# facebookresearch/spdl

Measured on AMD Instinct MI355X. Metric: images/sec device-resident JPEG→RGB224, 1/2/4/8×MI355X; % HBM roofline, higher is better.
Workload: dtype u8; 1 GPU; configs[1]: synthetic 480x640 q90 4:2:0 baseline JPEG resident in HBM -> RGB 224x224 u8 (scale bicubic decrease + centred pad, rgb24); global_batch=256, per_gpu_batch=256, distinct_images=32, lanes=4, hw_queues=4, entropy_threads=256, entropy_piece_bytes=131072

## Files before the change

### spdl_amd/csrc/hj_common.h

```cpp
#pragma once
#include <stddef.h>
#include <stdint.h>

#ifndef HJ_HD
#define HJ_HD __host__ __device__
#endif

namespace hj {

constexpr int kMaxComp = 4;

enum { kColorGray = 0, kColorYcbcr, kColorRgb, kColorCmyk, kColorYcck, kColorYcbcrk };
inline HJ_HD bool frame_color(int ncomp, const int32_t* h, const int32_t* v, const int* ids,
                              int adobe, int32_t* color) {
  bool all11 = true;
  for (int c = 0; c < ncomp; c++) all11 = all11 && h[c] == 1 && v[c] == 1;
  if (ncomp == 1) {
    *color = kColorGray;
  } else if (ncomp == 3) {
    const bool rgb = adobe == 0 || (ids[0] == 'R' && ids[1] == 'G' && ids[2] == 'B');
    if (rgb && !all11) return false;
    *color = rgb ? kColorRgb : kColorYcbcr;
  } else {
    if (!all11) return false;
    *color = adobe == 0 ? kColorCmyk : adobe == 2 ? kColorYcck : kColorYcbcrk;
  }
  return true;
}
constexpr int kMaxBpm = 10;
constexpr int kLutBits = 10;
constexpr int kLutSize = 1 << kLutBits;
constexpr int kDcBias = 1024;

constexpr int kMaxSlots = 2048;
constexpr int kRecPad = 4;
constexpr int kMaxEntropyThreads = 1024;

constexpr int kMaxPieces = 64;
constexpr int kChainGranules = 16;
constexpr int kChainHead = 32;
enum ChainSlot {
  kChG0 = 0, kChG1, kChL0, kChL1, kChT,
  kChE0, kChE1, kChB,
  kChDc = 8,
};
enum ChainTag : uint32_t { kTagRec1 = 1, kTagRec2 = 2, kTagDc = 3, kTagFail = 0xFA11u };
inline HJ_HD uint32_t slot_bits(uint32_t maxbits, int sub_bits, uint32_t budget = kMaxSlots) {
  uint32_t need = (uint32_t)(((uint64_t)maxbits + budget - 1) / budget);
  need = (need + 31) & ~31u;
  const uint32_t n = (uint32_t)sub_bits;
  return need > n ? need : n;
}

constexpr uint32_t kKindSlow = 0;
constexpr uint32_t kKindCode = 1;
constexpr uint32_t kKindFull = 2;
constexpr uint32_t kKindSub = 3;
constexpr int kSubBits = 16 - kLutBits;
#ifndef HJ_SUB_POOL
#define HJ_SUB_POOL 2048
#endif
constexpr int kSubPool = HJ_SUB_POOL;

#ifndef HJ_FUSED_THREADS
#define HJ_FUSED_THREADS 256
#endif
constexpr int kFusedThreads = HJ_FUSED_THREADS;
constexpr int kMaxSub = 16;
constexpr int kEntHiShift = 21;

inline HJ_HD uint32_t hj_entry(uint32_t kind, int len, int sym, bool is_dc, int v) {
  const int size = is_dc ? sym : (sym & 15);
  const int run = is_dc ? 0 : (sym >> 4);
  uint32_t zinc, coef = 0, bad = 0;
  if (is_dc || size) {
    zinc = (uint32_t)run + 1u;
    coef = 1;
  } else if (run == 15) {
    zinc = 16;
  } else {
    zinc = 64;
    bad = run != 0;
  }
  const uint32_t sz = kind == kKindFull ? 0u : (uint32_t)size;
  return ((uint32_t)len + sz) | (kind << 5) | (sz << 7) | (zinc << 12) | (coef << 19) | (bad << 20) |
         (((uint32_t)v & 0x7FFu) << kEntHiShift);
}

struct HuffTable {
  uint32_t lut[kLutSize];
  uint32_t sub[kMaxSub << kSubBits];
  int32_t nsub;
  int32_t long_slow;
  int32_t sub_lo;
  int32_t maxcode[18];
  int32_t valoff[17];
  uint8_t vals[256];
};

enum { kSwsX = 0, kSwsOne = 1, kSwsTwo = 2 };
enum SwsTable { kHlPos = 0, kHlCoef, kHcPos, kHcCoef, kVlPos, kVlCoef, kVcPos, kVcCoef, kVmode, kSwsTables };
struct SwsDesc {
  int32_t sw, sh;
  int32_t chr_w;
  int32_t full, gray;
  int32_t hl_taps, hc_taps, vl_taps, vc_taps;
  int32_t hl_size, hc_size, vl_size, vc_size;
  int32_t off[kSwsTables];
  int32_t rb;
  int32_t col_chunk;
  int32_t gbr;
  int32_t pre, pre_rl, pre_rc;
  int32_t yuv, hsub, vsub, chr_h;
};

struct ImageDesc {
  int64_t in_off;
  int64_t in_size;
  int64_t coef_off;
  int64_t plane_off[kMaxComp];
  int64_t seg_off;
  int64_t out_off;
  int64_t wt_off;
  int32_t seg_cap;
  int32_t width, height, ncomp;
  int32_t h_samp[kMaxComp], v_samp[kMaxComp];
  int32_t nblocks;
  int32_t plane_stride[kMaxComp];
  int32_t dx, dy, ow, oh;
  SwsDesc sws;
  int64_t ds_off;
  int32_t ds_cap;
  int32_t color;
  int64_t rec_off;
  int64_t rec_cap;
  int32_t pieces;
  int32_t chain_off;
  int32_t ds_wg0, idct_wg0;
  int32_t hs_wg0, hs_wgs;
  int32_t sws_wg0, sws_bands, sws_chunks;
  int64_t hbuf_off;
  int32_t refuse;
  int32_t idct_blocks;
  int32_t reg_mx0, reg_my0, reg_mw, reg_mh;
  uint32_t reg_mw_magic;
  int32_t win_x[kMaxComp], win_y[kMaxComp], win_w[kMaxComp], win_h[kMaxComp];
  int32_t src;
};

#ifndef HJ_SWS_LDS_KB
#define HJ_SWS_LDS_KB 32
#endif
constexpr int kSwsLdsBudget = HJ_SWS_LDS_KB * 1024;
constexpr int kSwsMaxCols = 256;
inline HJ_HD int sws_col_stride(int rows) { return 2 * (((rows + 5) >> 1) | 1); }

struct ImageInfo {
  int32_t status;
  int32_t width, height, ncomp, hmax, vmax, mcux, mcuy, bpm, nblocks, ri;
  int32_t scan_start;
  int32_t comp_h[kMaxComp], comp_v[kMaxComp];
  int32_t comp_bw[kMaxComp], comp_bh[kMaxComp];
  int32_t comp_w[kMaxComp], comp_hpx[kMaxComp];
  int32_t mcu_comp[kMaxBpm], mcu_dx[kMaxBpm], mcu_dy[kMaxBpm];
  int32_t dc_tab[kMaxComp], ac_tab[kMaxComp];
  uint16_t qt[kMaxComp][64];
  int32_t nseg;
  int32_t clean_len;
// ... 128 lines not shown
```

### spdl_amd/csrc/hj_kernels.hip

```cpp
#include <hip/hip_fp16.h>
#include <hip/hip_runtime.h>

#include "hj_common.h"
#include "hj_destuff.h"
#include "hj_idct.h"
#include "hj_launch.h"
#include "hj_sws_tile.h"

namespace hj {

__device__ __forceinline__ uint32_t rfl(uint32_t v) { return __builtin_amdgcn_readfirstlane(v); }


struct ParseScratch {
  ImageInfo info;
  uint16_t qt[4][64];
  uint8_t bits[8][17];
  uint8_t vals[8][256];
  int32_t have[8];
  int32_t qhave[4];
  int32_t maxcode[8][18];
  int32_t valoff[8][17];
  int32_t dqt_off[4], dqt_pq[4];
  int32_t dht_off[8], dht_n[8];
// ... 302 lines not shown
          k += s.bits[t][l];
          s.maxcode[t][l] = code - 1;
        } else {
          s.maxcode[t][l] = -1;
          s.valoff[t][l] = 0;
        }
        code <<= 1;
      }
      s.maxcode[t][17] = 0x7FFFFFFF;
    }
  }
  __syncthreads();
  HJ_PT();
  if (st != kOk) {
    if (tid == 0) infos[img] = s.info;
    return;
  }
  {
    const Bytes file{bytes + dd.in_off, (lds_u8*)hdr, nh};
    for (int i = tid; i < 8 * 256; i += blockDim.x) {
      const int t = i >> 8, k = i & 255;
      if (s.have[t]) s.vals[t][k] = k < s.dht_n[t] ? file[s.dht_off[t] + k] : 0;
    }
    for (int i = tid; i < 4 * 64; i += blockDim.x) {
      const int t = i >> 6, k = i & 63;
      if (s.qhave[t])
        s.qt[t][k] = s.dqt_pq[t] ? (uint16_t)((file[s.dqt_off[t] + 2 * k] << 8) |
                                              file[s.dqt_off[t] + 2 * k + 1])
                                 : file[s.dqt_off[t] + k];
    }
  }
  __syncthreads();
  HJ_PT();
  for (int i = tid; i < s.info.ncomp * 64; i += blockDim.x)
    s.info.qt[i / 64][i % 64] = s.qt[s.qtsel[i / 64]][i % 64];
  __syncthreads();
  if (s.info.multiscan) {
    if (tid == 0) infos[img] = s.info;
    return;
  }
  __shared__ int tab_nsub[8], tab_slow;
  if (tid == 0) tab_slow = 0;
  __syncthreads();
  if (tid < 8) {
    const int t = tid;
    int nsub = 0;
    if (s.have[t]) {
      uint32_t h = 2166136261u;
      for (int l = 1; l <= 16; l++) h = (h ^ s.bits[t][l]) * 16777619u;
      for (int k = 0; k < s.dht_n[t]; k++) h = (h ^ s.vals[t][k]) * 16777619u;
      s.info.tab_off[t] = s.dht_off[t] - 16;
      s.info.tab_n[t] = s.dht_n[t];
      s.info.tab_hash[t] = h;
      int p_lo = kLutSize, p_hi = -1;
      for (int l = kLutBits + 1; l <= 16; l++) {
        if (s.bits[t][l] == 0) continue;
        const int first = s.maxcode[t][l] - s.bits[t][l] + 1;
        p_lo = min(p_lo, first >> (l - kLutBits));
        p_hi = max(p_hi, s.maxcode[t][l] >> (l - kLutBits));
      }
      nsub = p_hi >= p_lo ? p_hi - p_lo + 1 : 0;
      if (nsub > kMaxSub) {
        atomicOr(&tab_slow, 1 << t);
        nsub = 0;
      }
    } else {
      s.info.tab_off[t] = 0;
      s.info.tab_n[t] = 0;
      s.info.tab_hash[t] = 0;
    }
    s.info.lut_ref[t] = img * 8 + t;
    tab_nsub[t] = nsub;
  }
  __syncthreads();
  if (tid == 0) {
    int ns = 0, seen = 0, subs = 0, slow = 0;
    for (int c = 0; c < s.info.ncomp; c++)
      for (int k = 0; k < 2; k++) {
        const int slot = k == 0 ? s.info.dc_tab[c] : 4 + s.info.ac_tab[c];
        if (!(seen & (1 << slot))) {
          ns++;
          subs += tab_nsub[slot];
          slow |= (tab_slow >> slot) & 1;
        }
        seen |= 1 << slot;
      }
    s.info.ent_wide = !(ns <= 4 && (subs << kSubBits) <= kSubPool && !slow);
  }
  __syncthreads();
  HJ_PT();
#if HJ_PARSE_PROF
  if (tid == 0)
    for (int i = 1; i < npt && i < 8; i++) s.info.sdiag[39 + i] = (int32_t)(pt[i] - pt[0]);
#endif
  static_assert(sizeof(ImageInfo) % 4 == 0, "ImageInfo copied in words");
  {
    const uint32_t* src = reinterpret_cast<const uint32_t*>(&s.info);
    uint32_t* dst = reinterpret_cast<uint32_t*>(infos + img);
    for (int i = tid; i < (int)(sizeof(ImageInfo) / 4); i += blockDim.x) dst[i] = src[i];
  }
}


__global__ void __launch_bounds__(256) lut_kernel(const uint8_t* __restrict__ bytes,
                                                  const ImageDesc* __restrict__ desc,
                                                  ImageInfo* __restrict__ infos,
                                                  HuffTable* __restrict__ luts) {
  __shared__ int first, same, maxcode[18], valoff[17];
  __shared__ uint8_t bits[17], vals[256];
  const int t = blockIdx.x, img = blockIdx.y, tid = threadIdx.x;
  const ImageInfo& in = infos[img];
  if (in.status != kOk || in.multiscan || in.tab_n[t] == 0) return;
  const uint32_t h = in.tab_hash[t];
  const int n = in.tab_n[t];
  const uint8_t* d = bytes + desc[img].in_off + in.tab_off[t];
  if (tid == 0) first = img;
  __syncthreads();
  for (int j = tid; j < img; j += blockDim.x) {
    const ImageInfo& o = infos[j];
    if (o.status == kOk && !o.multiscan && o.tab_n[t] == n && o.tab_hash[t] == h)
      atomicMin(&first, j);
  }
  __syncthreads();
  const int j = first;
  if (j < img) {
    if (tid == 0) same = 1;
    __syncthreads();
    const uint8_t* e = bytes + desc[j].in_off + infos[j].tab_off[t];
    for (int k = tid; k < 16 + n; k += blockDim.x)
      if (d[k] != e[k]) same = 0;
    __syncthreads();
    if (same) {
      if (tid == 0) infos[img].lut_ref[t] = j * 8 + t;
      return;
    }
  }
  if (tid < 16) bits[tid + 1] = d[tid];
  for (int k = tid; k < 256; k += blockDim.x) vals[k] = k < n ? d[16 + k] : 0;
  __syncthreads();
  if (tid == 0) {
    int code = 0, k = 0;
    for (int l = 1; l <= 16; l++) {
      if (bits[l]) {
        valoff[l] = k - code;
        code += bits[l];
        k += bits[l];
        maxcode[l] = code - 1;
      } else {
        maxcode[l] = -1;
        valoff[l] = 0;
      }
      code <<= 1;
    }
    maxcode[17] = 0x7FFFFFFF;
  }
  __syncthreads();
  HuffTable& T = luts[(size_t)img * 8 + t];
  const bool is_dc = t < 4;
  int p_lo = kLutSize, p_hi = -1;
  for (int l = kLutBits + 1; l <= 16; l++) {
    if (bits[l] == 0) continue;
    const int fc = maxcode[l] - bits[l] + 1;
    p_lo = min(p_lo, fc >> (l - kLutBits));
    p_hi = max(p_hi, maxcode[l] >> (l - kLutBits));
  }
  const int nsub = p_hi >= p_lo ? p_hi - p_lo + 1 : 0;
// ... 265 lines not shown
#pragma unroll
    for (int i = 0; i < 5; i++) atomicOr(q + i, x[i]);
  }
  __syncthreads();
  stage_to_global(out, stage, tk, tid);
  if (k == last) {
    const int clen = c.keep_pre + tk;
    if (tid < 64) out[tk + tid] = 0;
    if (tid == 0) {
      infos[img].clean_len = clen;
      infos[img].nseg = min(c.rst_pre + tr + 1, dd.seg_cap);
      sg[0] = 0;
    }
  }
}


typedef unsigned short hj_u16x2 __attribute__((ext_vector_type(2)));
__device__ __forceinline__ uint32_t pk_mul_lo16(uint32_t a, uint32_t b) {
  return __builtin_bit_cast(uint32_t,
                            __builtin_bit_cast(hj_u16x2, a) * __builtin_bit_cast(hj_u16x2, b));
}

constexpr int kMaxTabs = 2 * kMaxComp;
__constant__ uint8_t kSlotOrder[64] = {
    0,  4,  8,  16, 12, 1,  5,  9,  20, 24, 32, 28, 17, 13, 2,  6,  10, 21, 25, 36, 40, 48,
    44, 33, 29, 18, 14, 3,  7,  11, 22, 26, 37, 41, 52, 56, 60, 49, 45, 34, 30, 19, 15, 23,
    27, 38, 42, 53, 57, 61, 50, 46, 35, 31, 39, 43, 54, 58, 62, 51, 47, 55, 59, 63};
#ifndef HJ_WIN_WORDS
#define HJ_WIN_WORDS 12
#endif
constexpr int kWinWords = HJ_WIN_WORDS;

template <int NT, int NTAB>
struct EntShared {
  static constexpr int kTabs = NTAB;
  uint32_t lut[NTAB][kLutSize];
  uint32_t sub[kSubPool];
  int32_t maxcode[NTAB][18];
  int32_t valoff[NTAB][17];
  uint8_t vals[NTAB][256];
  uint32_t run_pos[NT];
  uint32_t run_zb[NT];
  uint32_t qdc[kMaxComp];
  union {
    uint32_t win[kWinWords][NT];
    struct {
      int32_t scan_flag[NT];
      int32_t scan_v[NT][kMaxComp];
      int32_t red[NT];
    } sc;
  };
  int32_t flag;
  int32_t err;
  uint64_t cmask[NT / 64], hmask[NT / 64];
  uint32_t chain_bits;
#if HJ_OWN_CHECK
  uint32_t own_viol;
#endif
  uint32_t chain_sweeps;
  uint32_t left_pos, left_zb;
  int32_t lb_ok, lb_blocks;
  int32_t lb_dc[kMaxComp];
  const HuffTable* gtab;
  int32_t gslot[kMaxTabs];
};
static_assert(sizeof(EntShared<512, 4>) <= 160 * 1024 / 2,
              "entropy LDS must allow 2 workgroups per CU");
static_assert(sizeof(EntShared<256, 4>) <= 160 * 1024 / 3,
              "entropy LDS must allow 3 workgroups per CU at 256 threads");

struct Dec {
  uint32_t wbit;
  uint32_t pos;
  uint32_t z;
  uint32_t bs;
};

struct TabMap {
  uint32_t dmap;
  uint32_t amap;
  uint32_t cmap;
  uint32_t bs_end;
  uint64_t soff;
};

template <int NT>
__device__ __forceinline__ void win_stage(uint32_t* win, const uint32_t* words, uint32_t wb) {
  static_assert(kWinWords % 4 == 0, "window is staged in uint4 units");
  typedef uint32_t u32x4 __attribute__((ext_vector_type(4), aligned(4)));
  const u32x4* src = reinterpret_cast<const u32x4*>(words + wb);
  u32x4 q[kWinWords / 4];
#pragma unroll
  for (int i = 0; i < kWinWords / 4; i++) q[i] = src[i];
#pragma unroll
  for (int i = 0; i < kWinWords / 4; i++) {
    win[(kWinWords - 1 - 4 * i) * NT] = __builtin_bswap32(q[i].x);
    win[(kWinWords - 2 - 4 * i) * NT] = __builtin_bswap32(q[i].y);
    win[(kWinWords - 3 - 4 * i) * NT] = __builtin_bswap32(q[i].z);
    win[(kWinWords - 4 - 4 * i) * NT] = __builtin_bswap32(q[i].w);
  }
}

template <int NT>
__device__ __forceinline__ void dec_init(Dec& d, uint32_t* win, const uint32_t* words, uint32_t p,
                                         uint32_t z, uint32_t bs) {
  d.wbit = p & ~31u;
  win_stage<NT>(win, words, p >> 5);
  d.pos = p;
  d.z = z;
  d.bs = bs;
}

template <int NT>
__device__ __forceinline__ uint32_t dec_peek(Dec& d, uint32_t* win, const uint32_t* words) {
  uint32_t rel = d.pos - d.wbit;
  if (__any(rel >= 32u * (kWinWords - 1))) {
    d.wbit = d.pos & ~31u;
    win_stage<NT>(win, words, d.pos >> 5);
    rel = d.pos - d.wbit;
  }
  const uint32_t* pw = win + (kWinWords - 2 - (int)(rel >> 5)) * NT;
  const uint64_t lohi = (uint64_t)pw[0] | ((uint64_t)pw[NT] << 32);
  return (uint32_t)((lohi << (rel & 31u)) >> 32);
}

__device__ __forceinline__ void dec_skip(Dec& d, uint32_t nbits) { d.pos += nbits; }

template <int NT>
__device__ __forceinline__ uint32_t dec_peek3(Dec& d, uint32_t* win, const uint32_t* words,
                                              uint64_t& p01, uint64_t& p12) {
  uint32_t rel = d.pos - d.wbit;
  if (__any(rel >= 32u * (kWinWords - 2))) {
    d.wbit = d.pos & ~31u;
    win_stage<NT>(win, words, d.pos >> 5);
    rel = d.pos - d.wbit;
  }
  const uint32_t* pw = win + (kWinWords - 3 - (int)(rel >> 5)) * NT;
  const uint32_t w2 = pw[0], w1 = pw[NT], w0 = pw[2 * NT];
  p01 = (uint64_t)w1 | ((uint64_t)w0 << 32);
  p12 = (uint64_t)w2 | ((uint64_t)w1 << 32);
  return rel & 31u;
}

__device__ __forceinline__ uint32_t tab_slot(const TabMap& m, const Dec& d, bool is_dc) {
  return __builtin_amdgcn_ubfe(is_dc ? m.dmap : m.amap, d.bs, 3);
}
__device__ __forceinline__ uint32_t next_bs(const TabMap& m, uint32_t bs) {
  return bs + 3u == m.bs_end ? 0u : bs + 3u;
}

template <class SH>
__device__ __attribute__((noinline)) uint32_t slow_symbol(const SH& S, int t, uint32_t hi,
                                                          bool is_dc) {
  const bool g = t >= SH::kTabs;
  const HuffTable* G = g ? S.gtab + S.gslot[t] : nullptr;
  const int tl = g ? 0 : t;
  const uint32_t w16 = hi >> 16;
  for (int l = 1; l <= 16; l++) {
    const int code = (int)(w16 >> (16 - l));
    if (code <= (g ? G->maxcode[l] : S.maxcode[tl][l])) {
      const int sym = g ? G->vals[G->valoff[l] + code] : S.vals[tl][S.valoff[tl][l] + code];
      if (is_dc && sym > 15) return 1;
      return hj_entry(kKindCode, l, sym, is_dc, 0);
    }
  }
  return 1;
}

template <bool SLOW, class SH>
__device__ __forceinline__ uint32_t lookup(const SH& S, uint32_t t, uint32_t hi, bool is_dc,
                                           uint64_t soff) {
  if constexpr (SLOW) {
    if (t >= (uint32_t)SH::kTabs) {
      const HuffTable& G = S.gtab[S.gslot[t]];
      uint32_t e = G.lut[hi >> (32 - kLutBits)];
      if (((e >> 5) & 3) == kKindSub)
        e = G.sub[((e >> kEntHiShift) << kSubBits) |
                  ((hi >> (32 - kLutBits - kSubBits)) & ((1u << kSubBits) - 1))];
      if (((e >> 5) & 3) == kKindSlow) e = slow_symbol(S, (int)t, hi, is_dc);
      return e;
    }
  }
  uint32_t e = S.lut[t][hi >> (32 - kLutBits)];
  if constexpr (!SLOW) {
    const uint32_t a2 = ((hi >> 16) + (uint32_t)(soff >> (16u * t))) & (uint32_t)(kSubPool - 1);
    const uint32_t e2 = S.sub[a2];
    return ((e >> 5) & 3) == kKindSub ? e2 : e;
  }
  if (((e >> 5) & 3) == kKindSub)
    e = S.sub[((e >> kEntHiShift) << kSubBits) |
              ((hi >> (32 - kLutBits - kSubBits)) & ((1u << kSubBits) - 1))];
  if constexpr (SLOW) {
    if (((e >> 5) & 3) == kKindSlow) e = slow_symbol(S, (int)t, hi, is_dc);
  }
  return e;
}

template <bool SLOW, class SH>
__device__ __forceinline__ uint32_t lookup_fast(const SH& S, uint32_t t, uint32_t hi,
                                                uint64_t soff) {
  if constexpr (SLOW) {
    if (t >= (uint32_t)SH::kTabs) {
      const HuffTable& G = S.gtab[S.gslot[t]];
      uint32_t e = G.lut[hi >> (32 - kLutBits)];
      if (((e >> 5) & 3) == kKindSub)
        e = G.sub[((e >> kEntHiShift) << kSubBits) |
                  ((hi >> (32 - kLutBits - kSubBits)) & ((1u << kSubBits) - 1))];
      return e;
    }
    uint32_t e = S.lut[t][hi >> (32 - kLutBits)];
    if (((e >> 5) & 3) == kKindSub)
      e = S.sub[((e >> kEntHiShift) << kSubBits) |
                ((hi >> (32 - kLutBits - kSubBits)) & ((1u << kSubBits) - 1))];
    return e;
  } else {
    return lookup<false>(S, t, hi, false, soff);
  }
}

template <int NT, bool SLOW, class SH>
__device__ int decode_state(const SH& S, Dec& d, uint32_t* win, const uint32_t* words,
                            const TabMap& m, const uint32_t end) {
  int nend = 0;
  const int open0 = d.z != 0u;
  while (d.pos < end) {
    uint64_t p01, p12;
    const uint32_t r = dec_peek3<NT>(d, win, words, p01, p12);
    uint32_t nbits;
    {
      const uint32_t hi = (uint32_t)((p01 << r) >> 32);
      const uint32_t z = d.z;
      const uint32_t t = tab_slot(m, d, z == 0u);
      const uint32_t e = lookup<SLOW>(S, t, hi, z == 0u, m.soff);
      nbits = e & 31u;
      dec_skip(d, nbits);
      const uint32_t zn = z + __builtin_amdgcn_ubfe(e, 12, 7);
      const bool bend = zn >= 64u;
      nend += bend ? 1 : 0;
      const uint32_t bsn = next_bs(m, d.bs);
      d.z = bend ? 0u : zn;
      d.bs = bend ? bsn : d.bs;
    }
    {
      const bool more = d.pos < end;
      const uint32_t r2 = r + nbits;
      const uint64_t pr = r2 < 32u ? p01 : p12;
      const uint32_t hi = (uint32_t)((pr << (r2 & 31u)) >> 32);
      const uint32_t z = d.z;
      const uint32_t t = tab_slot(m, d, z == 0u);
      const uint32_t e = lookup<SLOW>(S, t, hi, z == 0u, m.soff);
      const uint32_t n2 = more ? (e & 31u) : 0u;
      dec_skip(d, n2);
      const uint32_t zn = z + __builtin_amdgcn_ubfe(e, 12, 7);
      const bool bend = more && zn >= 64u;
      nend += bend ? 1 : 0;
      const uint32_t bsn = next_bs(m, d.bs);
      d.z = bend ? 0u : (more ? zn : z);
      d.bs = bend ? bsn : d.bs;
    }
  }
  return nend + (d.z != 0u ? 1 : 0) - open0;
}

template <int NT, bool SLOW, class SH>
__device__ void skip_open_block(const SH& S, Dec& d, uint32_t* win, const uint32_t* words,
                                const TabMap& m, const uint32_t seg_end) {
  while (d.z != 0u && d.pos < seg_end) {
    const uint32_t hi = dec_peek<NT>(d, win, words);
    const uint32_t z = d.z;
    const uint32_t e = lookup<SLOW>(S, tab_slot(m, d, false), hi, false, m.soff);
    const uint32_t nbits = e & 31u;
    dec_skip(d, nbits);
    const uint32_t zn = z + __builtin_amdgcn_ubfe(e, 12, 7);
    const bool bend = zn >= 64u;
    const uint32_t bsn = next_bs(m, d.bs);
    d.z = bend ? 0u : zn;
    d.bs = bend ? bsn : d.bs;
  }
}


__device__ __forceinline__ int sym_value(uint32_t e, uint32_t hi, uint32_t nbits, uint32_t sz) {
  const uint32_t raw = __builtin_amdgcn_ubfe(hi, 32u - nbits, sz);
  const uint32_t top = (uint32_t)__builtin_amdgcn_sbfe((int)raw, sz - 1u, 1);
  const uint32_t neg = ~top & ((1u << sz) - 1u);
  return ((int32_t)e >> kEntHiShift) + (int)(raw - neg);
}

#ifndef HJ_DESC_PAIRS
#define HJ_DESC_PAIRS 0
#endif
struct BlockOut {
  uint32_t* ents;
  uint2* bdesc;
  uint32_t cur;
  uint32_t last;
  uint32_t nblk;
  uint32_t bstart;
  int dcv;
  bool open;
  uint32_t pk[4];
#if HJ_DESC_PAIRS
  uint2 held;
  int hblk;
#endif
#if HJ_OWN_CHECK
  int lo, hi;
  uint32_t viol;
#endif
#if HJ_ABLATIONS
  bool no_list, no_desc;
#endif
};

__device__ __forceinline__ void put_entry(BlockOut& o, uint32_t e, bool put) {
  o.pk[0] = put ? o.pk[1] : o.pk[0];
  o.pk[1] = put ? o.pk[2] : o.pk[1];
  o.pk[2] = put ? o.pk[3] : o.pk[2];
  o.pk[3] = put ? e : o.pk[3];
#if HJ_ABLATIONS
  if (o.no_list) return;
#endif
  if (put && (o.cur & 3u) == 3u) {
    const uint32_t base = min(o.cur & ~3u, o.last & ~3u);
    *reinterpret_cast<uint4*>(o.ents + base) = make_uint4(o.pk[0], o.pk[1], o.pk[2], o.pk[3]);
  }
}

__device__ __forceinline__ void close_block(BlockOut& o, int blk) {
#if HJ_ABLATIONS
  if (o.no_desc) blk = -1;
#endif
  if ((uint32_t)blk < o.nblk) {
#if HJ_OWN_CHECK
    o.viol += (blk < o.lo || blk >= o.hi) ? 1u : 0u;
#endif
    const uint2 dv = make_uint2(o.bstart, (o.cur - o.bstart) | ((uint32_t)o.dcv << 16));
#if HJ_DESC_PAIRS
    uint2* p = o.bdesc + blk;
    const bool hi = ((uintptr_t)p & 8u) != 0;
    if (hi && o.hblk >= 0 && o.hblk == blk - 1) {
      *reinterpret_cast<uint4*>(p - 1) = make_uint4(o.held.x, o.held.y, dv.x, dv.y);
      o.hblk = -1;
    } else {
      if (o.hblk >= 0) o.bdesc[o.hblk] = o.held;
      if (hi) {
        *p = dv;
        o.hblk = -1;
      } else {
        o.held = dv;
        o.hblk = blk;
      }
    }
#else
    o.bdesc[blk] = dv;
#endif
  }
  o.open = false;
}

__device__ __forceinline__ void flush_desc(BlockOut& o) {
#if HJ_DESC_PAIRS
  if (o.hblk >= 0) o.bdesc[o.hblk] = o.held;
  o.hblk = -1;
#endif
}

__device__ __forceinline__ void flush_tail(BlockOut& o) {
  const uint32_t r = o.cur & 3u;
  if (r == 0u) return;
#if HJ_ABLATIONS
  if (o.no_list) return;
#endif
  const uint32_t base = min(o.cur & ~3u, o.last & ~3u);
  const uint32_t m1 = 0u - (uint32_t)(r == 1u), m2 = 0u - (uint32_t)(r == 2u);
  const uint32_t m3 = ~(m1 | m2);
  uint4 q;
  q.x = (o.pk[3] & m1) | (o.pk[2] & m2) | (o.pk[1] & m3);
  q.y = (o.pk[3] & m2) | (o.pk[2] & m3);
  q.z = o.pk[3];
  q.w = 0u;
  *reinterpret_cast<uint4*>(o.ents + base) = q;
}

template <int NT, bool SLOW, class SH>
__device__ int decode_write(const SH& S, Dec& d, uint32_t* win, const uint32_t* words,
                            const TabMap& m, const uint32_t end, const uint32_t seg_end,
                            const int seg_end_blk, BlockOut& o, int& nb, bool& done) {
  int rc = kOk;
  const int nb_entry = nb;
  auto fast_step = [&](const uint32_t hi) -> bool {
    const uint32_t z = d.z;
    const bool is_dc = z == 0;
    const uint32_t e = lookup<SLOW>(S, tab_slot(m, d, is_dc), hi, is_dc, m.soff);
    const uint32_t sz = __builtin_amdgcn_ubfe(e, 7, 5);
    const uint32_t nbits = e & 31u;
    const uint32_t zn = z + __builtin_amdgcn_ubfe(e, 12, 7);
    const bool coef = (e >> 19) & 1u;
    const uint32_t rules =
        ((64u - zn) & ((e & 0x80000u) << 12)) | ((e & 0x100060u) - 0x20u);
    if (rules > 0x40u) return false;
    const int v = sym_value(e, hi, nbits, sz);
    dec_skip(d, nbits);
    const bool ac = coef & !is_dc;
    put_entry(o, (uint32_t)v << 16 | (zn - 1u), ac);
    o.cur += ac ? 1u : 0u;
    o.bstart = is_dc ? o.cur : o.bstart;
    o.dcv = is_dc ? v : o.dcv;
    nb += is_dc ? 1 : 0;
    const bool bend = zn >= 64u;
    if (bend) close_block(o, nb - 1);
    const uint32_t bsn = next_bs(m, d.bs);
    d.z = bend ? 0u : zn;
    d.bs = bend ? bsn : d.bs;
    return true;
  };
  auto fast_stop = [&]() -> bool {
    const bool is_dc = d.z == 0u;
    return (is_dc & ((d.pos >= end) | (nb >= seg_end_blk))) | (d.pos + 32u > seg_end);
  };
  for (;;) {
    if (fast_stop()) break;
    uint64_t p01, p12;
    const uint32_t r = dec_peek3<NT>(d, win, words, p01, p12);
    const uint32_t pos0 = d.pos;
    if (!fast_step((uint32_t)((p01 << r) >> 32))) break;
    if (fast_stop()) break;
    const uint32_t r2 = r + (d.pos - pos0);
    const uint64_t pr = r2 < 32u ? p01 : p12;
    if (!fast_step((uint32_t)((pr << (r2 & 31u)) >> 32))) break;
  }
  o.open = d.z != 0u && nb > nb_entry;
  while (!done && rc == kOk && !(d.z == 0u && d.pos >= end)) {
    const uint32_t hi = dec_peek<NT>(d, win, words);
    const uint32_t z = d.z;
    const bool is_dc = z == 0;
    const uint32_t e = lookup<SLOW>(S, tab_slot(m, d, is_dc), hi, is_dc, m.soff);
    const bool valid = (e & 0x60u) != 0u;
    const uint32_t sz = __builtin_amdgcn_ubfe(e, 7, 5);
    const uint32_t nbits = e & 31u;
    const int v = sym_value(e, hi, nbits, sz);
    dec_skip(d, nbits);
    const uint32_t zinc = __builtin_amdgcn_ubfe(e, 12, 7);
    const bool coef = valid && ((e >> 19) & 1u);
    const bool bad = !valid || (coef && z + zinc > 64u) || ((e >> 20) & 1u);
    const bool past_a = nb > seg_end_blk || (nb == seg_end_blk && z == 0u);
    const bool good = coef && !bad;
    const bool stop = good && (is_dc ? nb : nb - 1) >= seg_end_blk;
    const bool wr = good && !stop;
    const uint32_t zn = valid ? z + zinc : z;
    if (wr && is_dc) {
      o.bstart = o.cur;
      o.dcv = v;
      o.open = true;
    }
    const bool put = wr && !is_dc;
    put_entry(o, (uint32_t)v << 16 | ((zn - 1u) & 63u), put);
    o.cur += put ? 1u : 0u;
    nb += (wr && is_dc) ? 1 : 0;
    const bool trunc = !bad && !stop && d.pos > seg_end;
    const bool past_b = nb > seg_end_blk || (nb == seg_end_blk && z == 0u);
    done = (bad && past_a) || stop || (trunc && past_b);
    rc = (bad && !past_a) ? kErrBadHuffman : ((trunc && !past_b) ? kErrTruncated : kOk);
    const bool bend = zn >= 64u;
    if (bend && !stop && o.open) close_block(o, nb - 1);
    const uint32_t bsn = next_bs(m, d.bs);
    d.z = bend ? 0u : zn;
    d.bs = bend ? bsn : d.bs;
  }
  if (o.open && d.z != 0u) close_block(o, nb - 1);
  return rc;
}

template <int NT, int NV, class SH>
__device__ void seg_scan(SH& S, int tid, int flag, const int (&v)[kMaxComp]) {
  S.sc.scan_flag[tid] = flag;
#pragma unroll
  for (int i = 0; i < NV; i++) S.sc.scan_v[tid][i] = v[i];
  __syncthreads();
  for (int off = 1; off < NT; off <<= 1) {
    int pf = 0, pv[NV];
    const bool take = tid >= off;
#pragma unroll
    for (int i = 0; i < NV; i++) pv[i] = take ? S.sc.scan_v[tid - off][i] : 0;
    if (take) pf = S.sc.scan_flag[tid - off];
    __syncthreads();
    if (take && !S.sc.scan_flag[tid]) {
#pragma unroll
      for (int i = 0; i < NV; i++) S.sc.scan_v[tid][i] += pv[i];
      S.sc.scan_flag[tid] = pf;
    }
    __syncthreads();
  }
}

typedef __attribute__((address_space(1))) unsigned long long hj_gu64;
__device__ __forceinline__ void gran_put(uint64_t* c, int i, uint32_t tag, uint32_t v) {
  __hip_atomic_store((hj_gu64*)(c + i), ((unsigned long long)tag << 32) | v, __ATOMIC_RELAXED,
                     __HIP_MEMORY_SCOPE_AGENT);
}
__device__ __forceinline__ uint64_t gran_get(const uint64_t* c, int i) {
  return __hip_atomic_load((hj_gu64*)(c + i), __ATOMIC_RELAXED, __HIP_MEMORY_SCOPE_AGENT);
}
constexpr int64_t kPollGapTicks = 100000;
struct WaitBound {
  int64_t last, idle;
  int sig;
};
__device__ __forceinline__ WaitBound wait_begin() { return WaitBound{wall_clock64(), 0, -1}; }
__device__ __forceinline__ bool wait_expired(WaitBound& w, int sig, int64_t limit) {
  const int64_t now = wall_clock64(), dt = now - w.last;
  w.last = now;
  if (sig != w.sig) {
    w.sig = sig;
    w.idle = 0;
    return false;
  }
  if (dt < kPollGapTicks) w.idle += dt;
  return w.idle >= limit;
}

__device__ __forceinline__ void chain_fail(uint64_t* rec, int tid) {
  if (tid < kChainGranules) gran_put(rec, tid, kTagFail, 0u);
}

template <class SH>
__device__ void chain_lookback(SH& S, const uint64_t* chain, int p, int lane, int64_t limit) {
  const uint64_t* rec = chain + (int64_t)(p - 1 - lane) * kChainGranules;
  const bool mine = lane < p;
  WaitBound wb = wait_begin();
  for (;;) {
    uint64_t r[8] = {};
    if (mine) {
#pragma unroll
      for (int i = 0; i < 8; i++) r[i] = gran_get(rec, i);
    }
    bool fail = false, has1 = mine, has2 = mine;
    int present = 0;
#pragma unroll
    for (int i = 0; i < 8; i++) {
      const uint32_t tag = (uint32_t)(r[i] >> 32);
      fail |= tag == kTagFail;
      present += __popcll(__ballot(tag != 0u));
      if (i < 5) has1 = has1 && tag == kTagRec1;
      else has2 = has2 && tag == kTagRec2;
    }
    if (__any(fail)) {
      if (lane == 0) S.lb_ok = -1;
      return;
    }
    const uint64_t m2 = __ballot(has2), m1 = __ballot(has1);
    if (m2 != 0) {
      const int lb = __builtin_ctzll(m2);
// ... 207 lines not shown
          "s_branch 2f\n"
          "3:\n\t"
          "s_mov_b32 %[be], 1\n"
          "2:"
          : [o] "+s"(o), [z] "+s"(z), [be] "=&s"(be), [t] "=&s"(t)
          : [nx] "v"(nx), [zi] "v"(zi), [lim] "s"(lim)
          : "scc");
      if (o >= 128u) {
        pos = wb + (o - 128u);
        const uint32_t r = pos - cbit;
        const uint64_t pr = ((uint64_t)cw[r >> 5] << 32) | cw[(r >> 5) + 1];
        const uint32_t hi = (uint32_t)((pr << (r & 31u)) >> 32);
        const bool isdc = z == 0u;
        const uint32_t e = rfl(lookup<kSlow>(
            S, __builtin_amdgcn_ubfe(isdc ? tm.dmap : tm.amap, bs, 3), hi, isdc, tm.soff));
        pos += e & 31u;
        const uint32_t zn = z + __builtin_amdgcn_ubfe(e, 12, 7);
        if (zn >= 64u) {
          nend++;
          bs = next_bs(tm, bs);
          z = 0u;
        } else {
          z = zn;
        }
        o = 64u;
        continue;
      }
      pos = wb + o;
      if (be) {
        nend++;
        bs = next_bs(tm, bs);
        z = 0u;
        o = 64u;
      }
    }
    if (lane == 0)
      sst[k] = make_uint4(p0, zb0,
                          (uint32_t)(nend + (z != 0u ? 1 : 0) - ((zb0 & 0xFFu) != 0u ? 1 : 0)), z);
    if (k + 1 == min(run_first(u) + K, nslots)) {
      if (lane == 0) {
        S.run_pos[u] = pos;
        S.run_zb[u] = z | (bs << 8);
      }
      u++;
    }
  }
  if (lane == 0) {
    atomicAdd(&S.chain_bits, pos - pos_in);
    atomicAdd(&S.chain_sweeps, 1u);
  }
}

template <int NT, int NTAB, bool kSlow>
__device__ __forceinline__ void entropy_image(EntShared<NT, NTAB>& S, const int img,
                              const uint8_t* __restrict__ clean, const uint32_t* __restrict__ segs,
                              const ImageDesc* __restrict__ desc, ImageInfo* __restrict__ infos,
                              const HuffTable* __restrict__ luts, uint32_t* __restrict__ ents,
                              uint2* __restrict__ bdesc, uint32_t* __restrict__ recs,
                              uint64_t* __restrict__ chain, const int piece,
                              const EntropyParams ep) {
  const int tid = threadIdx.x;
  const int ablate = HJ_ABLATIONS ? ep.ablate : 0;
  uint32_t* win = &S.win[0][tid];
  const ImageDesc dd = desc[img];
  const ImageInfo& in = infos[img];
  const int P = max(1, dd.pieces);
  uint64_t* crec = chain + kChainHead + dd.chain_off;
  uint64_t* myrec = crec + (int64_t)piece * kChainGranules;
  if (tid == 0) S.flag = (in.status != kOk || in.multiscan) ? 1 : 0;
  __syncthreads();
  if (S.flag) {
    if (P > 1) chain_fail(myrec, tid);
    return;
  }
  const int bpm = in.bpm, ri = in.ri, nmcu = in.mcux * in.mcuy;
  const int nblocks = in.nblocks;
  const uint32_t* words = reinterpret_cast<const uint32_t*>(clean + dd.in_off);
  const uint32_t* sg = segs + dd.seg_off;
  const int clean_len = in.clean_len;
  const int nseg_found = in.nseg;
  const int nseg = ri > 0 ? (nmcu + ri - 1) / ri : 1;

  uint32_t bcomp = 0;
  TabMap tm{0u, 0u, 0u, 0u, 0ull};
  {
    int slots[kMaxTabs], ns = 0, ldc[kMaxComp] = {}, lac[kMaxComp] = {};
    for (int c = 0; c < in.ncomp; c++) {
      const int want[2] = {in.dc_tab[c], 4 + in.ac_tab[c]};
      for (int k = 0; k < 2; k++) {
        int f = -1;
        for (int i = 0; i < ns; i++)
          if (slots[i] == want[k]) f = i;
        if (f < 0) {
          f = ns;
          slots[ns++] = want[k];
        }
        (k == 0 ? ldc : lac)[c] = f;
      }
    }
    if (tid == 0) S.gtab = luts;
    int pool = 0;
    for (int i = 0; i < ns; i++) {
      const int ref = in.lut_ref[slots[i]];
      if (i >= NTAB) {
        if (tid == 0) S.gslot[i] = ref;
        continue;
      }
      const HuffTable& T = luts[ref];
      const int nsub = T.nsub;
      const bool fits = (pool + nsub) << kSubBits <= kSubPool;
      const int base = pool;
      if (fits) pool += nsub;
      if (fits && nsub > 0)
        tm.soff |= (uint64_t)((uint32_t)((base - T.sub_lo) << kSubBits) & 0xFFFFu) << (16 * i);
      for (int k = tid; k < kLutSize; k += NT) {
        uint32_t e = T.lut[k];
        if ((e >> 5 & 3) == kKindSub) e = fits ? e + ((uint32_t)base << kEntHiShift) : 1u;
        S.lut[i][k] = e;
      }
      if (fits)
        for (int k = tid; k < nsub << kSubBits; k += NT)
          S.sub[(base << kSubBits) + k] = T.sub[k];
      if (tid < 18) S.maxcode[i][tid] = T.maxcode[tid];
      if (tid < 17) S.valoff[i][tid] = T.valoff[tid];
      for (int k = tid; k < 256; k += NT) S.vals[i][k] = T.vals[k];
    }
    if (tid < kMaxComp) S.qdc[tid] = in.qt[tid][0];
    for (int b = 0; b < bpm; b++) {
      const int c = in.mcu_comp[b];
      bcomp |= (uint32_t)c << (2 * b);
      tm.dmap |= (uint32_t)ldc[c] << (3 * b);
      tm.amap |= (uint32_t)lac[c] << (3 * b);
      tm.cmap |= (uint32_t)c << (3 * b);
    }
    tm.bs_end = 3u * (uint32_t)bpm;
    if (tid == 0) {
      S.err = kOk;
      S.chain_bits = 0;
      S.chain_sweeps = 0;
#if HJ_OWN_CHECK
      S.own_viol = 0;
#endif
    }
  }
  if (nseg_found < nseg) {
    if (tid == 0) infos[img].status = kErrBadRestart;
    if (P > 1) chain_fail(myrec, tid);
    return;
  }
  __syncthreads();

  const bool chained = P > 1 && ri == 0;
  const int seg_a = (P > 1 && !chained) ? (int)((int64_t)piece * nseg / P) : 0;
  const int seg_b = (P > 1 && !chained) ? (int)((int64_t)(piece + 1) * nseg / P) : nseg;
  const int pc = chained ? piece : 0;
  const int nruns = chained ? P * NT : NT;
  const uint32_t budget = (uint32_t)kMaxSlots * (chained ? P : 1);

  auto seg_start_bits = [&](int s) -> uint32_t { return sg[s] * 8u; };
  auto seg_end_bits = [&](int s) -> uint32_t {
    return (s + 1 < nseg_found ? sg[s + 1] : (uint32_t)clean_len) * 8u;
  };

  uint32_t maxbits = 0;
  for (int s = tid; s < nseg; s += NT) {
    const uint32_t a = seg_start_bits(s), e = seg_end_bits(s);
    maxbits = max(maxbits, e > a ? e - a : 0u);
  }
  S.sc.red[tid] = (int32_t)maxbits;
  __syncthreads();
  for (int off = NT / 2; off > 0; off >>= 1) {
    if (tid < off) S.sc.red[tid] = max(S.sc.red[tid], S.sc.red[tid + off]);
    __syncthreads();
  }
  maxbits = (uint32_t)S.sc.red[0];
  __syncthreads();
  const uint32_t N = slot_bits(maxbits, ep.sub_bits, budget);
  if ((int64_t)kMaxSlots * 8 * P > dd.rec_cap) {
    if (tid == 0) infos[img].status = kErrBadGeometry;
    if (P > 1) chain_fail(myrec, tid);
    return;
  }
  const int cmax = max(1, (int)((maxbits + N - 1) / N));
  const int seg_per_chunk = max(1, (int)(budget / (uint32_t)cmax));
  uint32_t* ents_img = ents + (size_t)dd.coef_off * 64;
  uint2* bdesc_img = bdesc + dd.coef_off;
  uint4* sst = reinterpret_cast<uint4*>(recs + dd.rec_off) +
              (chained ? 0 : (size_t)piece * kMaxSlots * 2);
  auto seg_first_blk = [&](int s) { return ri > 0 ? s * ri * bpm : 0; };
  auto seg_end_blk = [&](int s) { return ri > 0 ? min((s + 1) * ri, nmcu) * bpm : nblocks; };
  int rounds_total = 0;
  int64_t tph[4] = {0, 0, 0, 0}, dcfix = 0, chain_ticks = 0;
  int64_t tstamp = wall_clock64();

  for (int seg_lo = seg_a; seg_lo < seg_b; seg_lo += seg_per_chunk) {
    const int nsc = min(seg_per_chunk, seg_b - seg_lo);
    const int nslots = nsc * cmax;
    const int K = max((nslots + nruns - 1) / nruns, ep.min_run_slots);
    const int r0 = min((pc * NT + tid) * K, nslots), r1 = min(r0 + K, nslots);
    auto slot_seg = [&](int k) { return seg_lo + k / cmax; };
    auto slot_j = [&](int k) { return k % cmax; };
    auto slot_start = [&](int k) { return seg_start_bits(slot_seg(k)) + (uint32_t)slot_j(k) * N; };
    auto slot_end = [&](int k) {
      const uint32_t a = slot_start(k) + N, e = seg_end_bits(slot_seg(k));
      return a < e ? a : e;
    };
    auto slot_empty = [&](int k) {
      return slot_j(k) > 0 && slot_start(k) >= seg_end_bits(slot_seg(k));
    };
    auto slot_known = [&](int k) { return slot_j(k) == 0; };
    auto decode_k = [&](Dec& d, int k) {
      const uint32_t p0 = d.pos, zb0 = d.z | (d.bs << 8);
      const int nblk = decode_state<NT, kSlow>(S, d, win, words, tm, slot_end(k));
      sst[k] = make_uint4(p0, zb0, (uint32_t)nblk, d.z);
    };

// ... 173 lines not shown
      if (!chained || pass > 0) break;
      if (tid == 0) {
        uint32_t g0 = 0u, g1 = 0xFFFFFFFFu, l0 = 0u, l1 = 0u;
        if (t_last >= 0) {
          const uint4 q = sst[r0];
          g0 = q.x;
          g1 = q.y;
          l0 = S.run_pos[t_last];
          l1 = S.run_zb[t_last];
        }
        gran_put(myrec, kChG0, kTagRec1, g0);
        gran_put(myrec, kChG1, kTagRec1, g1);
        gran_put(myrec, kChL0, kTagRec1, l0);
        gran_put(myrec, kChL1, kTagRec1, l1);
        gran_put(myrec, kChT, kTagRec1, (uint32_t)blk_total);
        if (pc == 0) {
          gran_put(myrec, kChE0, kTagRec2, l0);
          gran_put(myrec, kChE1, kTagRec2, l1);
          gran_put(myrec, kChB, kTagRec2, (uint32_t)blk_total);
        }
        S.lb_ok = 1;
        S.lb_blocks = 0;
      }
      if (pc == 0) break;
      if (tid < 64) chain_lookback(S, crec, pc, tid, ep.handoff_ticks);
      __syncthreads();
      const int ok = S.lb_ok;
      if (ok < 0) {
        if (tid == 0 && ok == -2) infos[img].status = kErrHandoff;
        chain_fail(myrec, tid);
        return;
      }
      if (tid == 0) {
        bool wrong = false;
        if (t_last >= 0) {
          const uint4 q = sst[r0];
          wrong = q.x != S.left_pos || q.y != S.left_zb;
        }
        S.flag = wrong ? 1 : 0;
      }
      __syncthreads();
      const bool resync = S.flag != 0;
      __syncthreads();
      if (!resync) break;
    }
    if (chained) {
      if (pc > 0 && tid == 0) {
        const bool empty = t_last < 0;
        gran_put(myrec, kChE0, kTagRec2, empty ? S.left_pos : S.run_pos[t_last]);
        gran_put(myrec, kChE1, kTagRec2, empty ? S.left_zb : S.run_zb[t_last]);
        gran_put(myrec, kChB, kTagRec2, (uint32_t)(S.lb_blocks + blk_total));
      }
      __syncthreads();
      nb += S.lb_blocks;
      run_end_blk += S.lb_blocks;
    }
    {
      const int64_t t = wall_clock64();
      tph[2] += t - tstamp;
      tstamp = t;
    }
    int b0 = 0, b1 = 0;
    {
      int k0 = r0;
      while (k0 < r1 && slot_empty(k0)) k0++;
      if (k0 < r1) {
        b0 = max(0, slot_known(k0) ? seg_first_blk(slot_seg(k0)) : nb);
        b1 = min(min(run_end_blk, seg_end_blk(slot_seg(r1 - 1))), nblocks);
      }
    }
    if ((ablate & (kAblEntWrite | kAblEntDc)) && chained && tid < kMaxComp)
      gran_put(myrec, kChDc + tid, kTagDc, 0u);
    if (ablate & kAblEntWrite) continue;
    {
      int rc = kOk;
      bool done = false;
      bool have = false;
      BlockOut o;
      o.ents = ents_img;
      o.bdesc = bdesc_img;
      o.cur = (uint32_t)b0 * 64u;
      o.last = (uint32_t)nblocks * 64u - 1u;
      o.nblk = (uint32_t)nblocks;
#if HJ_ABLATIONS
      o.no_list = (ablate & kAblEntList) != 0;
      o.no_desc = (ablate & kAblEntDesc) != 0;
#endif
      o.bstart = o.cur;
      o.dcv = 0;
      o.open = false;
#if HJ_DESC_PAIRS
      o.hblk = -1;
      o.held = make_uint2(0u, 0u);
#endif
#if HJ_OWN_CHECK
      o.lo = b0;
      o.hi = b1;
      o.viol = 0u;
#endif
#pragma unroll
      for (uint32_t i = 0; i < 4; i++) o.pk[i] = 0u;
      Dec d;
      for (int k = r0; k < r1 && rc == kOk;) {
        const int s = slot_seg(k);
        const uint32_t s0 = seg_start_bits(s), se = seg_end_bits(s);
        const int jlast = se > s0 ? (int)((se - s0 - 1) / N) : 0;
        const int k2 = min(r1 - 1, (s - seg_lo) * cmax + jlast);
        if (k > k2) {
          have = false;
          k = min(r1, (s - seg_lo + 1) * cmax);
          continue;
        }
        if (slot_known(k)) {
          nb = seg_first_blk(s);
          done = false;
          dec_init<NT>(d, win, words, s0, 0, 0);
          have = true;
        } else if (!have) {
          const uint4 q = sst[k];
          dec_init<NT>(d, win, words, q.x, q.y & 0xFF, q.y >> 8);
          skip_open_block<NT, kSlow>(S, d, win, words, tm, se);
          have = true;
        }
        if (!done) {
          const int seb = seg_end_blk(s);
          const uint32_t pend = min(s0 + (uint32_t)(slot_j(k2) + 1) * N, se);
          rc = decode_write<NT, kSlow>(S, d, win, words, tm, pend, se, seb, o, nb, done);
          const bool last = (k2 + 1 >= nslots) || slot_j(k2 + 1) == 0 || pend >= se;
          if (rc == kOk && !done && last && (nb < seb || (nb == seb && d.z != 0)))
            rc = kErrTruncated;
        }
        k = k2 + 1;
      }
      flush_tail(o);
      flush_desc(o);
#if HJ_OWN_CHECK
      if (o.viol) atomicAdd(&S.own_viol, o.viol);
#endif
      if (rc != kOk) atomicCAS(&S.err, kOk, rc);
    }
    __syncthreads();
    {
      const int64_t t = wall_clock64();
      tph[3] += t - tstamp;
      tstamp = t;
    }
    if (ablate & kAblEntDc) continue;
    {
      const int rblk = ri > 0 ? ri * bpm : 0x7FFFFFFF;
      const int first_reset = ri > 0 ? (b0 + rblk - 1) / rblk * rblk : 0x7FFFFFFF;
      const int bs0 = b0 % bpm;
      int v[kMaxComp] = {}, flag = 0;
      constexpr int kG = 8;
      {
        int bs = bs0, reset = first_reset;
        for (int b = b0; b < b1; b += kG) {
          uint32_t ys[kG];
#pragma unroll
          for (int g = 0; g < kG; g++) ys[g] = bdesc_img[min(b + g, b1 - 1)].y;
#pragma unroll
          for (int g = 0; g < kG; g++) {
            if (b + g >= b1) break;
            if (b + g == reset) {
              flag = 1;
#pragma unroll
              for (int i = 0; i < kMaxComp; i++) v[i] = 0;
// ... 3315 lines not shown
```

Before: 594,300 images/sec.

## Micro-optimize Huffman hot loop: fixed sub-table slots, alignbit window, reversed block-slot map

Adds several entropy-decoder hot-loop tweaks, all on by default. Each table gets a fixed 512-entry sub-table slice addressed directly instead of through a packed offset. LUT entries that point to a sub-table become a single marker value. The second symbol's bit window comes from a single alignbit, and the step rules are recoded so one compare checks validity. Block-slot advance uses a reversed map with a min instead of compare-and-wrap, and the stop test is simplified. Together these cut ALU work per symbol, at the cost of sending images with large sub-tables to the slow path and of more complex bit encodings.

Result: faster. 613,700 images/sec (median of 6 runs) (+3.3%).

```diff
diff --git a/spdl_amd/csrc/hj_common.h b/spdl_amd/csrc/hj_common.h
--- a/spdl_amd/csrc/hj_common.h
+++ b/spdl_amd/csrc/hj_common.h
@@ -61,6 +61,34 @@
 #define HJ_SUB_POOL 2048
 #endif
 constexpr int kSubPool = HJ_SUB_POOL;
+#ifndef HJ_ENT_SUBADDR
+#define HJ_ENT_SUBADDR 1
+#endif
+#ifndef HJ_ENT_SUBMARK
+#define HJ_ENT_SUBMARK 1
+#endif
+#ifndef HJ_ENT_MORE
+#define HJ_ENT_MORE 1
+#endif
+#ifndef HJ_ENT_RULES
+#define HJ_ENT_RULES 1
+#endif
+#ifndef HJ_ENT_WIN2
+#define HJ_ENT_WIN2 1
+#endif
+#ifndef HJ_ENT_STOREBASE
+#define HJ_ENT_STOREBASE 1
+#endif
+#ifndef HJ_ENT_NEXTBS
+#define HJ_ENT_NEXTBS 1
+#endif
+#ifndef HJ_ENT_FASTSTOP
+#define HJ_ENT_FASTSTOP 1
+#endif
+constexpr int kSubShareBits = 9;
+constexpr int kSubShare = 1 << kSubShareBits;
+constexpr uint32_t kSubMark = kKindSub << 5;
+static_assert(!HJ_ENT_SUBADDR || 4 * kSubShare == kSubPool, "four slots share the pool evenly");
 
 #ifndef HJ_FUSED_THREADS
 #define HJ_FUSED_THREADS 256
@@ -83,7 +111,8 @@
     bad = run != 0;
   }
   const uint32_t sz = kind == kKindFull ? 0u : (uint32_t)size;
-  return ((uint32_t)len + sz) | (kind << 5) | (sz << 7) | (zinc << 12) | (coef << 19) | (bad << 20) |
+  const uint32_t b20 = HJ_ENT_RULES ? (uint32_t)(!coef && !bad) : bad;
+  return ((uint32_t)len + sz) | (kind << 5) | (sz << 7) | (zinc << 12) | (coef << 19) | (b20 << 20) |
          (((uint32_t)v & 0x7FFu) << kEntHiShift);
 }
 
diff --git a/spdl_amd/csrc/hj_kernels.hip b/spdl_amd/csrc/hj_kernels.hip
--- a/spdl_amd/csrc/hj_kernels.hip
+++ b/spdl_amd/csrc/hj_kernels.hip
@@ -408,6 +408,9 @@
           ns++;
           subs += tab_nsub[slot];
           slow |= (tab_slow >> slot) & 1;
+#if HJ_ENT_SUBADDR
+          slow |= tab_nsub[slot] > (kSubShare >> kSubBits);
+#endif
         }
         seen |= 1 << slot;
       }
@@ -839,6 +842,9 @@
   uint32_t amap;
   uint32_t cmap;
   uint32_t bs_end;
+#if HJ_ENT_NEXTBS
+  uint32_t rdmap, ramap;
+#endif
   uint64_t soff;
 };
 
@@ -900,11 +906,34 @@
   return rel & 31u;
 }
 
+__device__ __forceinline__ uint32_t win_next(uint32_t hi, uint32_t lo, uint32_t nbits) {
+  return __builtin_amdgcn_alignbit(hi, lo, 32u - nbits);
+}
+
 __device__ __forceinline__ uint32_t tab_slot(const TabMap& m, const Dec& d, bool is_dc) {
   return __builtin_amdgcn_ubfe(is_dc ? m.dmap : m.amap, d.bs, 3);
 }
 __device__ __forceinline__ uint32_t next_bs(const TabMap& m, uint32_t bs) {
   return bs + 3u == m.bs_end ? 0u : bs + 3u;
+}
+__device__ __forceinline__ void hot_flip(const TabMap& m, Dec& d) {
+#if HJ_ENT_NEXTBS
+  d.bs = m.bs_end - 3u - d.bs;
+#endif
+}
+__device__ __forceinline__ uint32_t hot_tab(const TabMap& m, const Dec& d, bool is_dc) {
+#if HJ_ENT_NEXTBS
+  return __builtin_amdgcn_ubfe(is_dc ? m.rdmap : m.ramap, d.bs, 3);
+#else
+  return tab_slot(m, d, is_dc);
+#endif
+}
+__device__ __forceinline__ uint32_t hot_next(const TabMap& m, uint32_t bs) {
+#if HJ_ENT_NEXTBS
+  return min(bs - 3u, m.bs_end - 3u);
+#else
+  return next_bs(m, bs);
+#endif
 }
 
 template <class SH>
@@ -941,9 +970,17 @@
   }
   uint32_t e = S.lut[t][hi >> (32 - kLutBits)];
   if constexpr (!SLOW) {
+#if HJ_ENT_SUBADDR
+    const uint32_t a2 = (t << kSubShareBits) | ((hi >> 16) & (uint32_t)(kSubShare - 1));
+#else
     const uint32_t a2 = ((hi >> 16) + (uint32_t)(soff >> (16u * t))) & (uint32_t)(kSubPool - 1);
+#endif
     const uint32_t e2 = S.sub[a2];
+#if HJ_ENT_SUBMARK
+    return e == kSubMark ? e2 : e;
+#else
     return ((e >> 5) & 3) == kKindSub ? e2 : e;
+#endif
   }
   if (((e >> 5) & 3) == kKindSub)
     e = S.sub[((e >> kEntHiShift) << kSubBits) |
@@ -981,42 +1018,67 @@
                             const TabMap& m, const uint32_t end) {
   int nend = 0;
   const int open0 = d.z != 0u;
+  hot_flip(m, d);
   while (d.pos < end) {
     uint64_t p01, p12;
     const uint32_t r = dec_peek3<NT>(d, win, words, p01, p12);
     uint32_t nbits;
+#if HJ_ENT_WIN2
+    const uint32_t hi0 = (uint32_t)((p01 << r) >> 32), lo0 = (uint32_t)((p12 << r) >> 32);
+#endif
     {
+#if HJ_ENT_WIN2
+      const uint32_t hi = hi0;
+#else
       const uint32_t hi = (uint32_t)((p01 << r) >> 32);
+#endif
       const uint32_t z = d.z;
-      const uint32_t t = tab_slot(m, d, z == 0u);
+      const uint32_t t = hot_tab(m, d, z == 0u);
       const uint32_t e = lookup<SLOW>(S, t, hi, z == 0u, m.soff);
       nbits = e & 31u;
       dec_skip(d, nbits);
       const uint32_t zn = z + __builtin_amdgcn_ubfe(e, 12, 7);
       const bool bend = zn >= 64u;
       nend += bend ? 1 : 0;
-      const uint32_t bsn = next_bs(m, d.bs);
+      const uint32_t bsn = hot_next(m, d.bs);
       d.z = bend ? 0u : zn;
       d.bs = bend ? bsn : d.bs;
     }
     {
       const bool more = d.pos < end;
+#if HJ_ENT_WIN2
+      const uint32_t hi = win_next(hi0, lo0, nbits);
+#else
       const uint32_t r2 = r + nbits;
       const uint64_t pr = r2 < 32u ? p01 : p12;
       const uint32_t hi = (uint32_t)((pr << (r2 & 31u)) >> 32);
+#endif
       const uint32_t z = d.z;
-      const uint32_t t = tab_slot(m, d, z == 0u);
+      const uint32_t t = hot_tab(m, d, z == 0u);
+#if HJ_ENT_MORE
+      const uint32_t es = lookup<SLOW>(S, t, hi, z == 0u, m.soff);
+      const uint32_t e = more ? es : 0u;
+      dec_skip(d, e & 31u);
+      const uint32_t zn = z + __builtin_amdgcn_ubfe(e, 12, 7);
+      const bool bend = zn >= 64u;
+      nend += bend ? 1 : 0;
+      const uint32_t bsn = hot_next(m, d.bs);
+      d.z = bend ? 0u : zn;
+      d.bs = bend ? bsn : d.bs;
+#else
       const uint32_t e = lookup<SLOW>(S, t, hi, z == 0u, m.soff);
       const uint32_t n2 = more ? (e & 31u) : 0u;
       dec_skip(d, n2);
       const uint32_t zn = z + __builtin_amdgcn_ubfe(e, 12, 7);
       const bool bend = more && zn >= 64u;
       nend += bend ? 1 : 0;
-      const uint32_t bsn = next_bs(m, d.bs);
+      const uint32_t bsn = hot_next(m, d.bs);
       d.z = bend ? 0u : (more ? zn : z);
       d.bs = bend ? bsn : d.bs;
-    }
-  }
+#endif
+    }
+  }
+  hot_flip(m, d);
   return nend + (d.z != 0u ? 1 : 0) - open0;
 }
 
@@ -1146,18 +1208,25 @@
                             const TabMap& m, const uint32_t end, const uint32_t seg_end,
                             const int seg_end_blk, BlockOut& o, int& nb, bool& done) {
   int rc = kOk;
+  hot_flip(m, d);
   const int nb_entry = nb;
   auto fast_step = [&](const uint32_t hi) -> bool {
     const uint32_t z = d.z;
     const bool is_dc = z == 0;
-    const uint32_t e = lookup<SLOW>(S, tab_slot(m, d, is_dc), hi, is_dc, m.soff);
+    const uint32_t e = lookup<SLOW>(S, hot_tab(m, d, is_dc), hi, is_dc, m.soff);
     const uint32_t sz = __builtin_amdgcn_ubfe(e, 7, 5);
     const uint32_t nbits = e & 31u;
     const uint32_t zn = z + __builtin_amdgcn_ubfe(e, 12, 7);
+#if HJ_ENT_RULES
+    const uint32_t lim = (e >> 13) & 0xC0u;
+    const bool coef = lim == 64u;
+    if (zn - 1u >= lim) return false;
+#else
     const bool coef = (e >> 19) & 1u;
     const uint32_t rules =
         ((64u - zn) & ((e & 0x80000u) << 12)) | ((e & 0x100060u) - 0x20u);
     if (rules > 0x40u) return false;
+#endif
     const int v = sym_value(e, hi, nbits, sz);
     dec_skip(d, nbits);
     const bool ac = coef & !is_dc;
@@ -1168,32 +1237,47 @@
     nb += is_dc ? 1 : 0;
     const bool bend = zn >= 64u;
     if (bend) close_block(o, nb - 1);
-    const uint32_t bsn = next_bs(m, d.bs);
+    const uint32_t bsn = hot_next(m, d.bs);
     d.z = bend ? 0u : zn;
     d.bs = bend ? bsn : d.bs;
     return true;
   };
+#if HJ_ENT_FASTSTOP
+  const uint32_t near_end = seg_end >= 31u ? seg_end - 31u : 0u;
+  auto fast_stop = [&]() -> bool {
+    const bool is_dc = d.z == 0u;
+    return (is_dc & ((d.pos >= end) | (nb >= seg_end_blk))) | (d.pos >= near_end);
+  };
+#else
   auto fast_stop = [&]() -> bool {
     const bool is_dc = d.z == 0u;
     return (is_dc & ((d.pos >= end) | (nb >= seg_end_blk))) | (d.pos + 32u > seg_end);
   };
+#endif
   for (;;) {
     if (fast_stop()) break;
     uint64_t p01, p12;
     const uint32_t r = dec_peek3<NT>(d, win, words, p01, p12);
     const uint32_t pos0 = d.pos;
+#if HJ_ENT_WIN2
+    const uint32_t hi0 = (uint32_t)((p01 << r) >> 32), lo0 = (uint32_t)((p12 << r) >> 32);
+    if (!fast_step(hi0)) break;
+    if (fast_stop()) break;
+    if (!fast_step(win_next(hi0, lo0, d.pos - pos0))) break;
+#else
     if (!fast_step((uint32_t)((p01 << r) >> 32))) break;
     if (fast_stop()) break;
     const uint32_t r2 = r + (d.pos - pos0);
     const uint64_t pr = r2 < 32u ? p01 : p12;
     if (!fast_step((uint32_t)((pr << (r2 & 31u)) >> 32))) break;
+#endif
   }
   o.open = d.z != 0u && nb > nb_entry;
   while (!done && rc == kOk && !(d.z == 0u && d.pos >= end)) {
     const uint32_t hi = dec_peek<NT>(d, win, words);
     const uint32_t z = d.z;
     const bool is_dc = z == 0;
-    const uint32_t e = lookup<SLOW>(S, tab_slot(m, d, is_dc), hi, is_dc, m.soff);
+    const uint32_t e = lookup<SLOW>(S, hot_tab(m, d, is_dc), hi, is_dc, m.soff);
     const bool valid = (e & 0x60u) != 0u;
     const uint32_t sz = __builtin_amdgcn_ubfe(e, 7, 5);
     const uint32_t nbits = e & 31u;
@@ -1201,7 +1285,8 @@
     dec_skip(d, nbits);
     const uint32_t zinc = __builtin_amdgcn_ubfe(e, 12, 7);
     const bool coef = valid && ((e >> 19) & 1u);
-    const bool bad = !valid || (coef && z + zinc > 64u) || ((e >> 20) & 1u);
+    const bool refused = HJ_ENT_RULES ? (e & 0x180000u) == 0u : ((e >> 20) & 1u) != 0u;
+    const bool bad = !valid || (coef && z + zinc > 64u) || refused;
     const bool past_a = nb > seg_end_blk || (nb == seg_end_blk && z == 0u);
     const bool good = coef && !bad;
     const bool stop = good && (is_dc ? nb : nb - 1) >= seg_end_blk;
@@ -1222,11 +1307,12 @@
     rc = (bad && !past_a) ? kErrBadHuffman : ((trunc && !past_b) ? kErrTruncated : kOk);
     const bool bend = zn >= 64u;
     if (bend && !stop && o.open) close_block(o, nb - 1);
-    const uint32_t bsn = next_bs(m, d.bs);
+    const uint32_t bsn = hot_next(m, d.bs);
     d.z = bend ? 0u : zn;
     d.bs = bend ? bsn : d.bs;
   }
   if (o.open && d.z != 0u) close_block(o, nb - 1);
+  hot_flip(m, d);
   return rc;
 }
 
@@ -1600,7 +1686,7 @@
   const int nseg = ri > 0 ? (nmcu + ri - 1) / ri : 1;
 
   uint32_t bcomp = 0;
-  TabMap tm{0u, 0u, 0u, 0u, 0ull};
+  TabMap tm{};
   {
     int slots[kMaxTabs], ns = 0, ldc[kMaxComp] = {}, lac[kMaxComp] = {};
     for (int c = 0; c < in.ncomp; c++) {
@@ -1626,19 +1712,29 @@
       }
       const HuffTable& T = luts[ref];
       const int nsub = T.nsub;
-      const bool fits = (pool + nsub) << kSubBits <= kSubPool;
+      constexpr bool kShared = HJ_ENT_SUBADDR && !kSlow;
+      const bool fits = kShared ? nsub << kSubBits <= kSubShare
+                                : (pool + nsub) << kSubBits <= kSubPool;
       const int base = pool;
-      if (fits) pool += nsub;
-      if (fits && nsub > 0)
+      if (fits && !kShared) pool += nsub;
+      if (!HJ_ENT_SUBADDR && fits && nsub > 0)
         tm.soff |= (uint64_t)((uint32_t)((base - T.sub_lo) << kSubBits) & 0xFFFFu) << (16 * i);
       for (int k = tid; k < kLutSize; k += NT) {
         uint32_t e = T.lut[k];
-        if ((e >> 5 & 3) == kKindSub) e = fits ? e + ((uint32_t)base << kEntHiShift) : 1u;
+        if ((e >> 5 & 3) == kKindSub) {
+          if (!fits) e = 1u;
+          else if (HJ_ENT_SUBMARK && !kSlow) e = kSubMark;
+          else e += (uint32_t)base << kEntHiShift;
+        }
         S.lut[i][k] = e;
       }
-      if (fits)
+      if (fits && kShared) {
+        for (int k = tid; k < nsub << kSubBits; k += NT)
+          S.sub[(i << kSubShareBits) + (((T.sub_lo << kSubBits) + k) & (kSubShare - 1))] = T.sub[k];
+      } else if (fits) {
         for (int k = tid; k < nsub << kSubBits; k += NT)
           S.sub[(base << kSubBits) + k] = T.sub[k];
+      }
       if (tid < 18) S.maxcode[i][tid] = T.maxcode[tid];
       if (tid < 17) S.valoff[i][tid] = T.valoff[tid];
       for (int k = tid; k < 256; k += NT) S.vals[i][k] = T.vals[k];
@@ -1650,6 +1746,10 @@
       tm.dmap |= (uint32_t)ldc[c] << (3 * b);
       tm.amap |= (uint32_t)lac[c] << (3 * b);
       tm.cmap |= (uint32_t)c << (3 * b);
+#if HJ_ENT_NEXTBS
+      tm.rdmap |= (uint32_t)ldc[c] << (3 * (bpm - 1 - b));
+      tm.ramap |= (uint32_t)lac[c] << (3 * (bpm - 1 - b));
+#endif
     }
     tm.bs_end = 3u * (uint32_t)bpm;
     if (tid == 0) {
@@ -1989,6 +2089,9 @@
       o.cur = (uint32_t)b0 * 64u;
       o.last = (uint32_t)nblocks * 64u - 1u;
       o.nblk = (uint32_t)nblocks;
+#if HJ_ENT_STOREBASE
+      asm volatile("" : "+v"(o.ents), "+v"(o.bdesc), "+v"(o.last), "+v"(o.nblk));
+#endif
 #if HJ_ABLATIONS
       o.no_list = (ablate & kAblEntList) != 0;
       o.no_desc = (ablate & kAblEntDesc) != 0;
```
